# tomisetsu/mochi-db

Hardware: AMD Instinct MI355X
Metric: verified grant signatures/sec (1/2/4/8 GPU) + % of INT32 VALU roofline (higher is better)
Workload: dtype u32

## Files before the change

mochi-db_amd/csrc/kara_dev.h:

```cpp
#pragma once
#include "fold.h"
#include "mont.h"

namespace mochi {

constexpr int kKH = kL / 2;
static_assert(2 * kKH == kL, "even limb count");

template <int AO, int BO, int K, int NA, int NB>
__device__ __forceinline__ uint32_t product_col(const uint32_t (&a)[NA], const uint32_t (&b)[NB], uint64_t& carry) {
  if constexpr (K == 2 * kKH - 1) {
    return (uint32_t)carry & kLimbMask;
  } else if constexpr (K == 2 * kKH) {
    return (uint32_t)(carry >> kLimbBits);
  } else {
    constexpr int lo = K - kKH + 1 > 0 ? K - kKH + 1 : 0;
    constexpr int hi = K < kKH - 1 ? K : kKH - 1;
    uint64_t acc = carry;
    static_for<lo, hi + 1>([&](auto ic) {
      constexpr int i = decltype(ic)::value;
      acc = mad64(a[AO + i], b[BO + K - i], acc);
      asm volatile("" ::"v"(acc));
    });
    carry = acc >> kLimbBits;
    return (uint32_t)acc & kLimbMask;
  }
}

template <int AO, int K, int NA>
__device__ __forceinline__ uint32_t square_col(uint32_t (&a)[NA], uint64_t& carry) {
  if constexpr (K == 2 * kKH - 1) {
    return (uint32_t)carry & kLimbMask;
  } else if constexpr (K == 2 * kKH) {
    return (uint32_t)(carry >> kLimbBits);
  } else {
    constexpr int lo = K - kKH + 1 > 0 ? K - kKH + 1 : 0;
    constexpr int xhi = K > 0 ? (K - 1) / 2 : -1;
    uint64_t acc = carry;
    static_for<lo, xhi + 1>([&](auto ic) {
      constexpr int i = decltype(ic)::value;
      acc = mad64(a[AO + i], a[AO + K - i], acc);
      asm volatile("" ::"v"(acc));
    });
    if constexpr ((K & 1) == 0) {
      acc = mad64(a[AO + (K >> 1)], a[AO + (K >> 1)], acc);
      if constexpr ((K >> 1) < kKH - 1) a[AO + (K >> 1)] += a[AO + (K >> 1)];
    }
    carry = acc >> kLimbBits;
    return (uint32_t)acc & kLimbMask;
  }
}

template <typename COL>
__device__ __forceinline__ void kara_middle(uint32_t (&t)[2 * kL], COL&& col) {
  uint64_t carry = 0;
  static_for<0, 2 * kKH + 1>([&](auto kc) {
    constexpr int k = decltype(kc)::value;
    t[kKH + k] = col(kc, carry);
    __builtin_amdgcn_sched_barrier(0);
  });
}

template <typename LOW, typename HIGH>
__device__ __forceinline__ void kara_combine(uint32_t (&t)[2 * kL], LOW&& low, HIGH&& high) {
  uint64_t cl = 0, ch = 0;
  static_for<0, 3 * kKH>([&](auto cc) {
    constexpr int c = decltype(cc)::value;
    if constexpr (c < kKH) {
      const uint32_t l = low(cc, cl);
      t[c] = l;
      t[kKH + c] -= l;
    } else if constexpr (c < kL) {
      const uint32_t l = low(cc, cl);
      const uint32_t h = high(std::integral_constant<int, c - kKH>{}, ch);
      const uint32_t q = l - h;
      t[c] += q;
      if constexpr (c >= kFoldF) t[c] ^= kFoldBias;
      t[kKH + c] -= q;
    } else {
      constexpr int m = c - kKH;
      const uint32_t h = high(std::integral_constant<int, m>{}, ch);
      t[c] -= h;
      t[c] ^= kFoldBias;
      if constexpr (m == kKH) {
        t[kKH + c] += h;
        t[kKH + c] ^= kFoldBias;
      } else {
        t[kKH + c] = h ^ kFoldBias;
      }
    }
    __builtin_amdgcn_sched_barrier(0);
  });
}

__device__ __forceinline__ void kara_square(uint32_t (&x)[kL], uint32_t (&t)[2 * kL]) {
  {
    uint32_t sx[kKH];
#pragma unroll
    for (int i = 0; i < kKH; i++) sx[i] = x[i] + x[kKH + i];
    kara_middle(t, [&](auto kc, uint64_t& carry) { return square_col<0, decltype(kc)::value>(sx, carry); });
  }
  kara_combine(
      t, [&](auto kc, uint64_t& carry) { return square_col<0, decltype(kc)::value>(x, carry); },
      [&](auto kc, uint64_t& carry) { return square_col<kKH, decltype(kc)::value>(x, carry); });
}

#ifndef MOCHI_KARA2
#define MOCHI_KARA2 0
#endif

template <int AO, int K, int N, int NA>
__device__ __forceinline__ uint32_t square_col_n(uint32_t (&a)[NA], uint64_t& carry) {
  if constexpr (K == 2 * N - 1) {
    return (uint32_t)carry & kLimbMask;
  } else if constexpr (K == 2 * N) {
    return (uint32_t)(carry >> kLimbBits);
  } else {
    constexpr int lo = K - N + 1 > 0 ? K - N + 1 : 0;
    constexpr int xhi = K > 0 ? (K - 1) / 2 : -1;
    uint64_t acc = carry;
    static_for<lo, xhi + 1>([&](auto ic) {
      constexpr int i = decltype(ic)::value;
      acc = mad64(a[AO + i], a[AO + K - i], acc);
      asm volatile("" ::"v"(acc));
    });
    if constexpr ((K & 1) == 0) {
      acc = mad64(a[AO + (K >> 1)], a[AO + (K >> 1)], acc);
      if constexpr ((K >> 1) < N - 1) a[AO + (K >> 1)] += a[AO + (K >> 1)];
    }
    carry = acc >> kLimbBits;
    return (uint32_t)acc & kLimbMask;
  }
}

template <int AO, int NA>
struct Square2 {
  static constexpr int N0 = 19, N1 = kKH - N0;
  uint32_t (&a)[NA];
  uint32_t s[N0];
  int32_t r[N0];
  uint64_t c0 = 0, c1 = 0, c2 = 0;
  int32_t cn = 0;
  __device__ __forceinline__ explicit Square2(uint32_t (&x)[NA]) : a(x) {
#pragma unroll
    for (int i = 0; i < N0; i++) s[i] = a[AO + i] + (i < N1 ? a[AO + N0 + i] : 0u);
  }
  template <int C>
  __device__ __forceinline__ uint32_t col() {
    int32_t p0 = 0, p1 = 0, p2 = 0;
    if constexpr (C <= 2 * N0) p0 = (int32_t)square_col_n<AO, C, N0>(a, c0);
    if constexpr (C - N0 >= 0 && C - N0 <= 2 * N1) p1 = (int32_t)square_col_n<AO + N0, C - N0, N1>(a, c1);
    if constexpr (C - N0 >= 0 && C - N0 <= 2 * N0) p2 = (int32_t)square_col_n<0, C - N0, N0>(s, c2);
    const int32_t rc = p0 - p1;
    int32_t v = rc + p2 + cn;
    if constexpr (C >= N0) v -= r[C % N0];
    r[C % N0] = rc;
    cn = v >> kLimbBits;
    return (uint32_t)v & kLimbMask;
  }
};

__device__ __forceinline__ void kara_square2_lockstep(uint32_t (&x)[kL], uint32_t (&t)[2 * kL]) {
  {
    uint32_t sx[kKH];
#pragma unroll
    for (int i = 0; i < kKH; i++) sx[i] = x[i] + x[kKH + i];
    kara_middle(t, [&](auto kc, uint64_t& carry) { return square_col<0, decltype(kc)::value>(sx, carry); });
  }
  Square2<0, kL> lo(x);
#if MOCHI_KARA2 == 5
  Square2<kKH, kL> hi(x);
  kara_combine(
      t, [&](auto kc, uint64_t&) { return lo.template col<decltype(kc)::value>(); },
      [&](auto kc, uint64_t&) { return hi.template col<decltype(kc)::value>(); });
#else
  kara_combine(
      t, [&](auto kc, uint64_t&) { return lo.template col<decltype(kc)::value>(); },
      [&](auto kc, uint64_t& carry) { return square_col<kKH, decltype(kc)::value>(x, carry); });
#endif
}

__device__ __forceinline__ void kara_square2(uint32_t (&x)[kL], uint32_t (&t)[2 * kL]) {
  {
    uint32_t sx[kKH];
#pragma unroll
    for (int i = 0; i < kKH; i++) sx[i] = x[i] + x[kKH + i];
    kara_middle(t, [&](auto kc, uint64_t& carry) { return square_col<0, decltype(kc)::value>(sx, carry); });
  }
  {
#if MOCHI_KARA2 == 3
    uint64_t cl = 0;
#else
    Square2<0, kL> lo(x);
#endif
    static_for<0, kL>([&](auto cc) {
      constexpr int c = decltype(cc)::value;
#if MOCHI_KARA2 == 3
      const uint32_t l = square_col<0, c>(x, cl);
#else
      const uint32_t l = lo.template col<c>();
#endif
      if constexpr (c < kKH) t[c] = l;
      else t[c] += l;
      t[kKH + c] -= l;
      __builtin_amdgcn_sched_barrier(0);
    });
  }
  {
#if MOCHI_KARA2 >= 2
    uint64_t ch = 0;
#else
    Square2<kKH, kL> hi(x);
#endif
    static_for<0, kL>([&](auto mc) {
      constexpr int m = decltype(mc)::value;
#if MOCHI_KARA2 >= 2
      const uint32_t h = square_col<kKH, m>(x, ch);
#else
      const uint32_t h = hi.template col<m>();
#endif
      t[kKH + m] -= h;
      if constexpr (m <= kKH) t[kL + m] += h;
      else t[kL + m] = h;
      __builtin_amdgcn_sched_barrier(0);
    });
  }
#pragma unroll
  for (int k = kFoldF; k < 2 * kL; k++) t[k] ^= kFoldBias;
}

__device__ __forceinline__ void kara_product(const uint32_t (&x)[kL], const uint32_t (&y)[kL], uint32_t (&t)[2 * kL]) {
  {
    uint32_t sx[kKH], sy[kKH];
#pragma unroll
    for (int i = 0; i < kKH; i++) {
      sx[i] = x[i] + x[kKH + i];
      sy[i] = y[i] + y[kKH + i];
    }
    kara_middle(t, [&](auto kc, uint64_t& carry) { return product_col<0, 0, decltype(kc)::value>(sx, sy, carry); });
  }
  kara_combine(
      t, [&](auto kc, uint64_t& carry) { return product_col<0, 0, decltype(kc)::value>(x, y, carry); },
      [&](auto kc, uint64_t& carry) { return product_col<kKH, kKH, decltype(kc)::value>(x, y, carry); });
}

}
```

mochi-db_amd/csrc/rsa_final.hip:

```cpp
#include "fold_dev.h"
#include "rsa_common.h"

#include <cstdlib>

#ifndef MOCHI_FINAL_DYN
#define MOCHI_FINAL_DYN 0
#endif

#ifndef MOCHI_FINAL_STAMPS
#define MOCHI_FINAL_STAMPS 0
#endif

namespace mochi {
#if MOCHI_FINAL_STAMPS
__device__ unsigned long long g_final_stamps[4096][6];
#endif
namespace {

struct FStamps {
  uint64_t load = 0, prod = 0, fold = 0, check = 0, n = 0;
};

__device__ __forceinline__ uint64_t fstamp() {
#if MOCHI_FINAL_STAMPS
  __builtin_amdgcn_sched_barrier(0);
  const uint64_t t = __builtin_amdgcn_s_memtime();
  __builtin_amdgcn_sched_barrier(0);
  return t;
#else
  return 0;
#endif
}

#ifndef MOCHI_FINAL_WAIT
#define MOCHI_FINAL_WAIT 1
#endif

struct FinalOps {
  uint4 sr[16];
  uint32_t z[kL];
  uint32_t hw[8];
  uint32_t g, fl, d;
};

__device__ __forceinline__ void final_load(uint32_t slot, uint32_t g_lead, const uint32_t* __restrict__ perm,
                                           uint32_t n_slots, const uint8_t* __restrict__ sig,
                                           const uint32_t* __restrict__ zin, const uint32_t* __restrict__ lead,
                                           const uint8_t* __restrict__ flags, FinalOps& o) {
  o.g = slot < n_slots ? perm[slot] : 0xFFFFFFFFu;
  const uint32_t gg = o.g != 0xFFFFFFFFu ? o.g : g_lead;
  o.d = lead ? lead[gg] : gg;
  o.fl = flags[gg];
  const uint4* s128 = (const uint4*)(sig + (size_t)gg * MOCHI_RSA_BYTES);
#pragma unroll
  for (int q = 0; q < 16; q++) o.sr[q] = s128[q];
  const gchar* zp = (const gchar*)zin;
  const uint32_t zoff = slot * 4u;
  const size_t zstride = (size_t)n_slots * 4u;
#pragma unroll
  for (int j = 0; j < kL; j++) {
    o.z[j] = *(const guint*)(zp + zoff);
    zp += zstride;
    asm volatile("" : "+s"(zp));
  }
}

__device__ __forceinline__ void final_load_digest(const uint32_t* __restrict__ digest, uint32_t n_dist, FinalOps& o) {
#pragma unroll
  for (int i = 0; i < 8; i++) o.hw[i] = digest[(size_t)(7 - i) * n_dist + o.d];
}

__device__ __forceinline__ void final_slot(FinalOps& o, uint32_t key, uint32_t g_lead,
                                           const KeyEntry* __restrict__ keys, const FoldKey* __restrict__ fold,
                                           const uint32_t* __restrict__ digest, const uint32_t* __restrict__ lead,
                                           uint32_t n_dist, uint8_t* __restrict__ flags, const v4i* w,
                                           FStamps& st) {
  const uint32_t g = o.g;
  const bool active = g != 0xFFFFFFFFu;
  if (__ballot(active) == 0) return;
  const uint64_t t1 = fstamp();
  const KeyEntry* ke = keys + key;
  const cptr n = as_const(ke->n);
  uint32_t sv[kL];
  {
    uint32_t wd[64];
#pragma unroll
    for (int q = 0; q < 16; q++) {
      wd[63 - 4 * q] = bswap32(o.sr[q].x);
      wd[62 - 4 * q] = bswap32(o.sr[q].y);
      wd[61 - 4 * q] = bswap32(o.sr[q].z);
      wd[60 - 4 * q] = bswap32(o.sr[q].w);
    }
    words_to_limbs(wd, sv);
  }
  int32_t br = 0;
#pragma unroll
  for (int j = 0; j < kL; j++) br = ((int32_t)sv[j] - (int32_t)n[j] - br) < 0 ? 1 : 0;
  asm volatile("" : "+v"(br));
  const bool s_lt_n = br != 0;
  uint32_t (&x)[kL] = o.z;
  uint32_t t[2 * kL];
  kara_product(x, sv, t);
  const uint64_t t2 = fstamp();
  uint32_t hl[kHL];
  {
    const uint32_t (&hw)[8] = o.hw;
#pragma unroll
    for (int j = 0; j < kHL; j++) {
      const int bit = j * kLimbBits, wi = bit >> 5, sh = bit & 31;
      const uint64_t v = ((uint64_t)(wi + 1 < 8 ? hw[wi + 1] : 0u) << 32) | hw[wi];
      hl[j] = (uint32_t)(v >> sh) & kLimbMask;
    }
  }
  fold_reduce<true, true>(t, x, w + (threadIdx.x & 63), as_const(fold[key].cnc), hl);
  const uint64_t t3 = fstamp();
  cptr nn = n;
  asm volatile("" : "+s"(nn));
  const uint32_t n0inv = *as_const(&ke->n0inv);
  const uint32_t m = (x[0] * n0inv) & kLimbMask;
  uint64_t c = mad64(m, nn[0], x[0]) >> kLimbBits;
  uint32_t diff = 0;
#pragma unroll
  for (int k = 1; k < kL; k++) {
    const uint64_t acc = mad64(m, nn[k], x[k] + c);
    diff |= ((uint32_t)acc & kLimbMask) ^ nn[k - 1];
    c = acc >> kLimbBits;
  }
  diff |= c != (uint64_t)nn[kL - 1] ? 1u : 0u;
  if (active) {
    const bool ok = s_lt_n && diff == 0;
    flags[g] = (uint8_t)(o.fl | (ok ? MOCHI_GRANT_SIG_OK : 0));
  }
#if MOCHI_FINAL_STAMPS
  const uint64_t t4 = fstamp();
  st.prod += t2 - t1;
  st.fold += t3 - t2;
  st.check += t4 - t3;
  st.n++;
#else
  (void)t1, (void)t2, (void)t3, (void)st;
#endif
}

__global__ __launch_bounds__(256, 1) void k_rsa_final(const uint32_t* __restrict__ perm, uint32_t n_slots,
                                                       const uint8_t* __restrict__ sig,
                                                       const uint16_t* __restrict__ signer,
                                                       const KeyEntry* __restrict__ keys,
                                                       const FoldKey* __restrict__ fold,
                                                       const uint32_t* __restrict__ zin,
                                                       const uint32_t* __restrict__ digest,
                                                       const uint32_t* __restrict__ lead, uint32_t n_dist,
                                                       uint8_t* __restrict__ flags, uint32_t* __restrict__ ctr) {
  __shared__ v4i w[kFoldImgBytes / 16];
  FStamps st;
  const uint64_t t_begin = fstamp();
  for_groups(perm, n_slots, signer, fold, w, [&](uint32_t base, uint32_t key, uint32_t g_lead) {
#pragma unroll 1
    for (uint32_t h = 0; h < kBucketAlign; h += 256) {
      FinalOps o;
      const uint64_t t0 = fstamp();
      final_load(base + h + threadIdx.x, g_lead, perm, n_slots, sig, zin, lead, flags, o);
#if MOCHI_FINAL_STAMPS == 2 || (MOCHI_FINAL_WAIT && !MOCHI_FINAL_STAMPS)
      asm volatile("s_waitcnt vmcnt(0)" ::: "memory");
#endif
      final_load_digest(digest, n_dist, o);
#if MOCHI_FINAL_STAMPS
      st.load += fstamp() - t0;
#endif
      (void)t0;
      final_slot(o, key, g_lead, keys, fold, digest, lead, n_dist, flags, w, st);
    }
  }, MOCHI_FINAL_DYN ? ctr : nullptr);
#if MOCHI_FINAL_STAMPS
  const uint64_t t_end = fstamp();
  const uint32_t wv = (blockIdx.x * blockDim.x + threadIdx.x) >> 6;
  if ((threadIdx.x & 63) == 0 && wv < 4096) {
    g_final_stamps[wv][0] = st.load;
    g_final_stamps[wv][1] = st.prod;
    g_final_stamps[wv][2] = st.fold;
    g_final_stamps[wv][3] = st.check;
    g_final_stamps[wv][4] = st.n;
    g_final_stamps[wv][5] = t_end - t_begin;
  }
#else
  (void)t_begin;
#endif
}

__global__ __launch_bounds__(256, 1) void k_rsa_final_lat(const uint32_t* __restrict__ perm, uint32_t n_slots,
                                                           const uint8_t* __restrict__ sig,
                                                           const uint16_t* __restrict__ signer,
                                                           const KeyEntry* __restrict__ keys,
                                                           const FoldKey* __restrict__ fold,
                                                           const uint32_t* __restrict__ zin,
                                                           const uint32_t* __restrict__ digest,
                                                           const uint32_t* __restrict__ lead, uint32_t n_dist,
                                                           uint8_t* __restrict__ flags) {
  __shared__ v4i w[kFoldImgBytes / 16];
  __shared__ uint32_t xr[kLatRows][kLatChunk];
  const uint32_t wv = __builtin_amdgcn_readfirstlane(threadIdx.x >> 6), lane = threadIdx.x & 63;
  const uint32_t base = blockIdx.x * kLatChunk;
  if (base >= n_slots) return;
  const uint32_t g_lead = __builtin_amdgcn_readfirstlane(perm[base]);
  if (g_lead == 0xFFFFFFFFu) return;
  const uint32_t key = __builtin_amdgcn_readfirstlane((uint32_t)signer[g_lead]);
  {
    const v4i* src = (const v4i*)fold[key].img;
    for (uint32_t i = threadIdx.x; i < kFoldImgBytes / 16; i += blockDim.x) w[i] = src[i];
  }
  const bool two = __builtin_amdgcn_readfirstlane(base + 32 < n_slots && perm[base + 32] != 0xFFFFFFFFu);
  const uint32_t slot = base + lane;
  const uint32_t g = slot < n_slots ? perm[slot] : 0xFFFFFFFFu;
  const bool active = g != 0xFFFFFFFFu;
  const uint32_t gg = active ? g : g_lead;
  const uint32_t fl = flags[gg];
  uint32_t z[kL], sv[kL];
#pragma unroll
  for (int j = 0; j < kL; j++) z[j] = zin[(size_t)j * n_slots + (slot < n_slots ? slot : base)];
  {
    uint32_t wd[64];
    load_sig_words(sig, gg, wd);
    words_to_limbs(wd, sv);
  }
  __syncthreads();
  uint32_t lv[kL];
  if (wv == 0) {
    uint64_t carry = 0;
    static_for<0, kL>([&](auto kc) {
      constexpr int k = decltype(kc)::value;
      lv[k] = product_col<0, 0, k>(z, sv, carry);
    });
  } else if (wv == 1) {
    uint32_t hv[kL];
    uint64_t carry = 0;
    static_for<0, kL>([&](auto kc) {
      constexpr int k = decltype(kc)::value;
      hv[k] = product_col<kKH, kKH, k>(z, sv, carry);
    });
#pragma unroll
    for (int k = 0; k < kL; k++) xr[k][lane] = hv[k];
  } else if (wv == 2) {
    uint32_t sz[kKH], ss[kKH];
#pragma unroll
    for (int i = 0; i < kKH; i++) {
      sz[i] = z[i] + z[kKH + i];
      ss[i] = sv[i] + sv[kKH + i];
    }
    uint32_t mv[kL + 1];
    uint64_t carry = 0;
    static_for<0, kL + 1>([&](auto kc) {
      constexpr int k = decltype(kc)::value;
      mv[k] = product_col<0, 0, k>(sz, ss, carry);
    });
#pragma unroll
    for (int k = 0; k <= kL; k++) xr[kL + k][lane] = mv[k];
  }
  __syncthreads();
  if (wv == 0) {
    uint32_t t[2 * kL], hv[kL];
#pragma unroll
    for (int k = 0; k <= kL; k++) t[kKH + k] = xr[kL + k][lane];
#pragma unroll
    for (int k = 0; k < kL; k++) hv[k] = xr[k][lane];
    kara_combine(
        t, [&](auto kc, uint64_t&) { return lv[decltype(kc)::value]; },
        [&](auto kc, uint64_t&) { return hv[decltype(kc)::value]; });
#pragma unroll
    for (int k = 0; k < 2 * kL; k++) xr[k][lane] = t[k];
  }
  uint32_t hl[kHL];
  {
    const uint32_t d = lead ? lead[gg] : gg;
    uint32_t hw[8];
#pragma unroll
    for (int i = 0; i < 8; i++) hw[i] = digest[(size_t)(7 - i) * n_dist + d];
#pragma unroll
    for (int j = 0; j < kHL; j++) {
      const int bit = j * kLimbBits, wi = bit >> 5, sh = bit & 31;
      const uint64_t v = ((uint64_t)(wi + 1 < 8 ? hw[wi + 1] : 0u) << 32) | hw[wi];
      hl[j] = (uint32_t)(v >> sh) & kLimbMask;
    }
  }
  __syncthreads();
  const v4i* wl = w + lane;
  cptr cn = as_const(fold[key].cnc);
  asm volatile("" : "+s"(cn));
  if (two) {
    if (wv == 0) lat_fold<0, true, true>(wl, cn, xr, lane, hl);
    else if (wv == 1) lat_fold<1, true, true>(wl, cn, xr, lane, hl);
    else if (wv == 2) lat_fold<2, true, true>(wl, cn, xr, lane, hl);
    else lat_fold<3, true, true>(wl, cn, xr, lane, hl);
  } else {
    if (wv == 0) lat_fold<0, false, true>(wl, cn, xr, lane, hl);
    else if (wv == 1) lat_fold<1, false, true>(wl, cn, xr, lane, hl);
    else if (wv == 2) lat_fold<2, false, true>(wl, cn, xr, lane, hl);
    else lat_fold<3, false, true>(wl, cn, xr, lane, hl);
  }
  __syncthreads();
  if (wv != 0) return;
  uint32_t x[kL];
  {
    int pq[2 * kL];
#pragma unroll
    for (int i = 0; i < 2 * kL; i++) pq[i] = (int)xr[i][lane];
    int64_t carry = 0;
#pragma unroll
    for (int q = 0; q < kL; q++) {
      const int64_t v = mad_i64(pq[2 * q + 1], 65536, mad_i64(pq[2 * q], 1, carry));
      x[q] = (uint32_t)v & kLimbMask;
      carry = v >> kLimbBits;
    }
  }
  const KeyEntry* ke = keys + key;
  const cptr n = as_const(ke->n);
  int32_t br = 0;
#pragma unroll
  for (int j = 0; j < kL; j++) br = ((int32_t)sv[j] - (int32_t)n[j] - br) < 0 ? 1 : 0;
  const uint32_t n0inv = *as_const(&ke->n0inv);
  const uint32_t m = (x[0] * n0inv) & kLimbMask;
  uint64_t c = mad64(m, n[0], x[0]) >> kLimbBits;
  uint32_t diff = 0;
#pragma unroll
  for (int k = 1; k < kL; k++) {
    const uint64_t acc = mad64(m, n[k], x[k] + c);
    diff |= ((uint32_t)acc & kLimbMask) ^ n[k - 1];
    c = acc >> kLimbBits;
  }
  diff |= c != (uint64_t)n[kL - 1] ? 1u : 0u;
  if (active) {
    const bool ok = br != 0 && diff == 0;
    flags[g] = (uint8_t)(fl | (ok ? MOCHI_GRANT_SIG_OK : 0));
  }
}

static bool final_lat_off() {
  static const bool off = [] {
    const char* e = getenv("MOCHI_NO_FINAL_LAT");
    return e && e[0] == '1';
  }();
  return off;
}

}

void launch_rsa_final(const LaunchArgs& a, const uint32_t* lead, uint32_t n_dist, hipStream_t st, bool latency) {
  if (a.dbg_y) {
    launch_rsa_raw(a, st);
    return;
  }
  if (latency && !final_lat_off()) {
    const uint32_t chunks = (a.n_slots + kLatChunk - 1) / kLatChunk;
    if (chunks)
      hipLaunchKernelGGL(k_rsa_final_lat, dim3(chunks), dim3(256), 0, st, a.perm, a.n_slots, a.sig, a.signer, a.keys,
                         a.fold, a.xbuf, a.digest, lead, n_dist, a.flags);
    return;
  }
  const uint32_t blocks = fold_grid(a.n_slots);
  if (!blocks) return;
  hipLaunchKernelGGL(k_rsa_final, dim3(blocks), dim3(256), 0, st, a.perm, a.n_slots, a.sig, a.signer, a.keys, a.fold,
                     a.xbuf, a.digest, lead, n_dist, a.flags, a.total + kTotFinalGroup);
}

}

#if MOCHI_FINAL_STAMPS
extern "C" int mochi_debug_final_stamps(unsigned long long* out, unsigned n_waves) {
  if (n_waves > 4096) n_waves = 4096;
  return hipMemcpyFromSymbol(out, HIP_SYMBOL(mochi::g_final_stamps), 48 * (size_t)n_waves, 0, hipMemcpyDeviceToHost) ==
                 hipSuccess
             ? 0
             : -1;
}
#endif
```

Measured before the change: 366.8 million.

## Split final RSA kernel into two phase-staggered wave groups with LDS-parked limbs

Replaces the final verification kernel with a 512-thread version. Two halves of the block run staggered with barriers, so one half's Karatsuba low/high product overlaps the other's fold-reduce and check. To cut register pressure, the low product limbs are parked in LDS rows through inline ds_write/ds_read with immediate offsets and reloaded before folding. The kernel also uses static contiguous group assignment per block instead of the dynamic counter and prefetches the next group's key, at the cost of extra barriers, more LDS use, and sensitivity to kBucketAlign matching the block size.

```diff
diff --git a/mochi-db_amd/csrc/kara_dev.h b/mochi-db_amd/csrc/kara_dev.h
--- a/mochi-db_amd/csrc/kara_dev.h
+++ b/mochi-db_amd/csrc/kara_dev.h
@@ -244,4 +244,101 @@
       [&](auto kc, uint64_t& carry) { return product_col<kKH, kKH, decltype(kc)::value>(x, y, carry); });
 }
 
-}
+constexpr int kParkLimbs = 28;
+constexpr int kParkStride = (int)kBucketAlign * 4;
+static_assert(kParkLimbs % 7 == 0 && kParkLimbs <= kKH, "parked limbs are read back seven at a time");
+static_assert((kParkLimbs - 1) * kParkStride < 65536, "row offsets fit the DS instruction's immediate");
+
+template <int ROW>
+__device__ __forceinline__ void park_put(uint32_t park, uint32_t v) {
+  asm volatile("ds_write_b32 %0, %1 offset:%2" ::"v"(park), "v"(v), "n"(ROW * kParkStride) : "memory");
+}
+
+template <int R0>
+__device__ __forceinline__ void park_get7(uint32_t park, uint32_t (&v)[7]) {
+  asm volatile(
+      "ds_read_b32 %0, %7 offset:%8\n\t"
+      "ds_read_b32 %1, %7 offset:%9\n\t"
+      "ds_read_b32 %2, %7 offset:%10\n\t"
+      "ds_read_b32 %3, %7 offset:%11\n\t"
+      "ds_read_b32 %4, %7 offset:%12\n\t"
+      "ds_read_b32 %5, %7 offset:%13\n\t"
+      "ds_read_b32 %6, %7 offset:%14\n\t"
+      "s_waitcnt lgkmcnt(0)"
+      : "=&v"(v[0]), "=&v"(v[1]), "=&v"(v[2]), "=&v"(v[3]), "=&v"(v[4]), "=&v"(v[5]), "=&v"(v[6])
+      : "v"(park), "n"(R0 * kParkStride), "n"((R0 + 1) * kParkStride), "n"((R0 + 2) * kParkStride),
+        "n"((R0 + 3) * kParkStride), "n"((R0 + 4) * kParkStride), "n"((R0 + 5) * kParkStride),
+        "n"((R0 + 6) * kParkStride)
+      : "memory");
+}
+
+__device__ __forceinline__ void park_reload(uint32_t park, uint32_t (&t)[2 * kL]) {
+  static_for<0, kParkLimbs / 7>([&](auto bc) {
+    constexpr int b = decltype(bc)::value;
+    uint32_t v[7];
+    park_get7<7 * b>(park, v);
+#pragma unroll
+    for (int j = 0; j < 7; j++) t[7 * b + j] = v[j];
+  });
+}
+
+__device__ __forceinline__ void kara_consume_lh(uint32_t (&x)[kL], uint32_t (&y)[kL], uint32_t (&t)[2 * kL],
+                                                uint32_t park) {
+  {
+    uint64_t cl = 0, ch = 0;
+    static_for<0, kL>([&](auto cc) {
+      constexpr int c = decltype(cc)::value;
+      uint32_t l = product_col<0, 0, c>(x, y, cl);
+      uint32_t h = product_col<kKH, kKH, c>(x, y, ch);
+      asm volatile("" : "+v"(l), "+v"(h));
+      if constexpr (c < kParkLimbs) park_put<c>(park, l);
+      else t[c] = l;
+      t[kL + c] = h;
+      if constexpr (c >= kKH - 1 && c - (kKH - 1) < kKH) {
+        constexpr int i = c - (kKH - 1);
+        x[i] += x[kKH + i];
+        y[i] += y[kKH + i];
+      }
+      __builtin_amdgcn_sched_barrier(0);
+    });
+  }
+  static_for<kKH, kL>([&](auto kc) {
+    constexpr int k = decltype(kc)::value;
+    constexpr int j = k - kKH;
+    const uint32_t q = t[k] - t[k + kKH];
+    t[k + kKH] = 0u - q - t[k + kL];
+    if constexpr (k + kL > kKH + kL) t[k + kL] ^= kFoldBias;
+    if constexpr (j >= kParkLimbs) t[k] = q - t[j];
+    else t[k] = q;
+    asm volatile("" : "+v"(t[k]), "+v"(t[k + kKH]), "+v"(t[k + kL]));
+  });
+  static_for<0, kParkLimbs / 7>([&](auto bc) {
+    constexpr int b = decltype(bc)::value;
+    uint32_t v[7];
+    park_get7<7 * b>(park, v);
+#pragma unroll
+    for (int j = 0; j < 7; j++) t[kKH + 7 * b + j] -= v[j];
+  });
+  __builtin_amdgcn_sched_barrier(0);
+}
+
+__device__ __forceinline__ void kara_consume_m(uint32_t (&x)[kL], uint32_t (&y)[kL], uint32_t (&t)[2 * kL]) {
+  {
+    uint64_t cm = 0;
+    static_for<0, 2 * kKH + 1>([&](auto mc) {
+      constexpr int m = decltype(mc)::value;
+      t[kKH + m] += product_col<0, 0, m>(x, y, cm);
+      if constexpr (kKH + m >= kFoldF) t[kKH + m] ^= kFoldBias;
+      asm volatile("" : "+v"(t[kKH + m]));
+      __builtin_amdgcn_sched_barrier(0);
+    });
+  }
+}
+
+__device__ __forceinline__ void kara_product_consume(uint32_t (&x)[kL], uint32_t (&y)[kL], uint32_t (&t)[2 * kL],
+                                                     uint32_t park) {
+  kara_consume_lh(x, y, t, park);
+  kara_consume_m(x, y, t);
+}
+
+}
diff --git a/mochi-db_amd/csrc/rsa_final.hip b/mochi-db_amd/csrc/rsa_final.hip
--- a/mochi-db_amd/csrc/rsa_final.hip
+++ b/mochi-db_amd/csrc/rsa_final.hip
@@ -9,6 +9,10 @@
 
 #ifndef MOCHI_FINAL_STAMPS
 #define MOCHI_FINAL_STAMPS 0
+#endif
+
+#ifndef MOCHI_FINAL_TWO
+#define MOCHI_FINAL_TWO 1
 #endif
 
 namespace mochi {
@@ -43,6 +47,7 @@
   uint32_t g, fl, d;
 };
 
+template <bool FLAGS = true>
 __device__ __forceinline__ void final_load(uint32_t slot, uint32_t g_lead, const uint32_t* __restrict__ perm,
                                            uint32_t n_slots, const uint8_t* __restrict__ sig,
                                            const uint32_t* __restrict__ zin, const uint32_t* __restrict__ lead,
@@ -50,7 +55,7 @@
   o.g = slot < n_slots ? perm[slot] : 0xFFFFFFFFu;
   const uint32_t gg = o.g != 0xFFFFFFFFu ? o.g : g_lead;
   o.d = lead ? lead[gg] : gg;
-  o.fl = flags[gg];
+  if constexpr (FLAGS) o.fl = flags[gg];
   const uint4* s128 = (const uint4*)(sig + (size_t)gg * MOCHI_RSA_BYTES);
 #pragma unroll
   for (int q = 0; q < 16; q++) o.sr[q] = s128[q];
@@ -70,6 +75,7 @@
   for (int i = 0; i < 8; i++) o.hw[i] = digest[(size_t)(7 - i) * n_dist + o.d];
 }
 
+#if !MOCHI_FINAL_TWO
 __device__ __forceinline__ void final_slot(FinalOps& o, uint32_t key, uint32_t g_lead,
                                            const KeyEntry* __restrict__ keys, const FoldKey* __restrict__ fold,
                                            const uint32_t* __restrict__ digest, const uint32_t* __restrict__ lead,
@@ -142,6 +148,183 @@
 #endif
 }
 
+#endif
+
+#if MOCHI_FINAL_TWO
+__device__ __forceinline__ uint32_t lane_id() {
+  uint32_t tid = threadIdx.x;
+  asm volatile("" : "+v"(tid));
+  return tid;
+}
+
+__device__ __forceinline__ void final_fold_check(uint32_t (&t)[2 * kL], const FinalOps& o, uint32_t key,
+                                                 const KeyEntry* __restrict__ keys, const FoldKey* __restrict__ fold,
+                                                 uint8_t* __restrict__ flags, const v4i* w, uint32_t park,
+                                                 FStamps& st) {
+  const uint64_t t2 = fstamp();
+  uint32_t hl[kHL];
+#pragma unroll
+  for (int j = 0; j < kHL; j++) {
+    const int bit = j * kLimbBits, wi = bit >> 5, sh = bit & 31;
+    const uint64_t v = ((uint64_t)(wi + 1 < 8 ? o.hw[wi + 1] : 0u) << 32) | o.hw[wi];
+    hl[j] = (uint32_t)(v >> sh) & kLimbMask;
+  }
+  park_reload(park, t);
+  uint32_t x[kL];
+  fold_reduce<true, true>(t, x, w + (lane_id() & 63), as_const(fold[key].cnc), hl);
+  const uint64_t t3 = fstamp();
+  const KeyEntry* ke = keys + key;
+  cptr nn = as_const(ke->n);
+  asm volatile("" : "+s"(nn));
+  const uint32_t n0inv = *as_const(&ke->n0inv);
+  const uint32_t m = (x[0] * n0inv) & kLimbMask;
+  uint64_t c = mad64(m, nn[0], x[0]) >> kLimbBits;
+  uint32_t diff = 0;
+#pragma unroll
+  for (int k = 1; k < kL; k++) {
+    const uint64_t acc = mad64(m, nn[k], x[k] + c);
+    diff |= ((uint32_t)acc & kLimbMask) ^ nn[k - 1];
+    c = acc >> kLimbBits;
+  }
+  diff |= c != (uint64_t)nn[kL - 1] ? 1u : 0u;
+  if (o.g != 0xFFFFFFFFu) {
+    flags[o.g] = (uint8_t)(o.fl | (diff == 0 ? MOCHI_GRANT_SIG_OK : 0));
+  }
+#if MOCHI_FINAL_STAMPS
+  st.fold += t3 - t2;
+  st.check += fstamp() - t3;
+  st.n++;
+#else
+  (void)t2, (void)t3, (void)st;
+#endif
+}
+
+__device__ __forceinline__ void phase_barrier() {
+  __builtin_amdgcn_sched_barrier(0);
+  __builtin_amdgcn_s_barrier();
+  __builtin_amdgcn_sched_barrier(0);
+}
+
+__global__ __launch_bounds__(512, 1) void k_rsa_final(const uint32_t* __restrict__ perm, uint32_t n_slots,
+                                                       const uint8_t* __restrict__ sig,
+                                                       const uint16_t* __restrict__ signer,
+                                                       const KeyEntry* __restrict__ keys,
+                                                       const FoldKey* __restrict__ fold,
+                                                       const uint32_t* __restrict__ zin,
+                                                       const uint32_t* __restrict__ digest,
+                                                       const uint32_t* __restrict__ lead, uint32_t n_dist,
+                                                       uint8_t* __restrict__ flags, uint32_t* __restrict__ ctr) {
+  __shared__ v4i w[kFoldImgBytes / 16];
+  __shared__ uint32_t park_rows[kParkLimbs * kBucketAlign];
+  FStamps st;
+  const uint64_t t_begin = fstamp();
+  auto park_of = [&](uint32_t tid) {
+    return (uint32_t)(uintptr_t)(__attribute__((address_space(3))) uint32_t*)(park_rows + tid);
+  };
+  const bool lag = __builtin_amdgcn_readfirstlane(threadIdx.x >> 6) >= 4;
+  const uint32_t n_groups = (n_slots + kBucketAlign - 1) / kBucketAlign;
+  uint32_t grp = (uint32_t)((uint64_t)blockIdx.x * n_groups / gridDim.x);
+  const uint32_t g_end = (uint32_t)((uint64_t)(blockIdx.x + 1) * n_groups / gridDim.x);
+  uint32_t g_lead = 0xFFFFFFFFu;
+  while (grp < g_end && (g_lead = __builtin_amdgcn_readfirstlane(perm[grp * kBucketAlign])) == 0xFFFFFFFFu) grp++;
+  if (grp >= g_end) return;
+  uint32_t key = __builtin_amdgcn_readfirstlane((uint32_t)signer[g_lead]);
+  auto stage = [&](uint32_t k) {
+    typedef __attribute__((address_space(1))) v4i gv4i;
+    const gchar* src = (const gchar*)fold[k].img;
+#pragma unroll 1
+    for (uint32_t i = lane_id(); i < kFoldImgBytes / 16; i += kBucketAlign) w[i] = *(const gv4i*)(src + i * 16u);
+    __syncthreads();
+  };
+  stage(key);
+  if (lag) phase_barrier();
+  bool key_changed = false;
+  for (;;) {
+    if (!lag && key_changed) {
+      phase_barrier();
+      stage(key);
+    }
+    FinalOps o;
+    final_load<false>(grp * kBucketAlign + threadIdx.x, g_lead, perm, n_slots, sig, zin, lead, flags, o);
+    uint32_t nxt = grp + 1, n_lead = 0xFFFFFFFFu;
+    while (nxt < g_end && (n_lead = __builtin_amdgcn_readfirstlane(perm[nxt * kBucketAlign])) == 0xFFFFFFFFu) nxt++;
+    const bool more = nxt < g_end;
+    const uint32_t n_key = more ? __builtin_amdgcn_readfirstlane((uint32_t)signer[n_lead]) : key;
+    const uint64_t t0 = fstamp();
+    asm volatile("s_waitcnt vmcnt(0)" ::: "memory");
+    const uint64_t t1 = fstamp();
+    if (__ballot(o.g != 0xFFFFFFFFu) != 0) {
+      uint32_t sv[kL];
+      {
+        uint32_t wd[64];
+#pragma unroll
+        for (int q = 0; q < 16; q++) {
+          wd[63 - 4 * q] = bswap32(o.sr[q].x);
+          wd[62 - 4 * q] = bswap32(o.sr[q].y);
+          wd[61 - 4 * q] = bswap32(o.sr[q].z);
+          wd[60 - 4 * q] = bswap32(o.sr[q].w);
+        }
+        words_to_limbs(wd, sv);
+      }
+      const cptr n = as_const(keys[key].n);
+      int32_t br = 0;
+#pragma unroll
+      for (int j = 0; j < kL; j++) br = ((int32_t)sv[j] - (int32_t)n[j] - br) < 0 ? 1 : 0;
+      if (br == 0) o.g = 0xFFFFFFFFu;
+      asm volatile("" : "+v"(o.g));
+      uint32_t t[2 * kL];
+      kara_consume_lh(o.z, sv, t, park_of(lane_id()));
+      final_load_digest(digest, n_dist, o);
+      o.fl = flags[o.g != 0xFFFFFFFFu ? o.g : g_lead];
+#if MOCHI_FINAL_STAMPS
+      st.load += t1 - t0;
+      st.prod += fstamp() - t1;
+#endif
+      __builtin_amdgcn_sched_barrier(0);
+      phase_barrier();
+      const uint64_t t1m = fstamp();
+      kara_consume_m(o.z, sv, t);
+#if MOCHI_FINAL_STAMPS
+      st.prod += fstamp() - t1m;
+#else
+      (void)t1m;
+#endif
+      __builtin_amdgcn_s_setprio(1);
+      final_fold_check(t, o, key, keys, fold, flags, w, park_of(lane_id()), st);
+      __builtin_amdgcn_s_setprio(0);
+    } else {
+      phase_barrier();
+    }
+    (void)t0, (void)t1;
+    phase_barrier();
+    if (!more) break;
+    if (lag && n_key != key) {
+      stage(n_key);
+      phase_barrier();
+    }
+    key_changed = n_key != key;
+    grp = nxt;
+    key = n_key;
+    g_lead = n_lead;
+  }
+  if (!lag) phase_barrier();
+#if MOCHI_FINAL_STAMPS
+  const uint64_t t_end = fstamp();
+  const uint32_t wv = (blockIdx.x * blockDim.x + threadIdx.x) >> 6;
+  if ((threadIdx.x & 63) == 0 && wv < 4096) {
+    g_final_stamps[wv][0] = st.load;
+    g_final_stamps[wv][1] = st.prod;
+    g_final_stamps[wv][2] = st.fold;
+    g_final_stamps[wv][3] = st.check;
+    g_final_stamps[wv][4] = st.n;
+    g_final_stamps[wv][5] = t_end - t_begin;
+  }
+#else
+  (void)t_begin;
+#endif
+  (void)ctr;
+}
+#else
 __global__ __launch_bounds__(256, 1) void k_rsa_final(const uint32_t* __restrict__ perm, uint32_t n_slots,
                                                        const uint8_t* __restrict__ sig,
                                                        const uint16_t* __restrict__ signer,
@@ -187,6 +370,8 @@
 #endif
 }
 
+#endif
+
 __global__ __launch_bounds__(256, 1) void k_rsa_final_lat(const uint32_t* __restrict__ perm, uint32_t n_slots,
                                                            const uint8_t* __restrict__ sig,
                                                            const uint16_t* __restrict__ signer,
@@ -357,7 +542,7 @@
   }
   const uint32_t blocks = fold_grid(a.n_slots);
   if (!blocks) return;
-  hipLaunchKernelGGL(k_rsa_final, dim3(blocks), dim3(256), 0, st, a.perm, a.n_slots, a.sig, a.signer, a.keys, a.fold,
+  hipLaunchKernelGGL(k_rsa_final, dim3(blocks), dim3(MOCHI_FINAL_TWO ? kBucketAlign : 256), 0, st, a.perm, a.n_slots, a.sig, a.signer, a.keys, a.fold,
                      a.xbuf, a.digest, lead, n_dist, a.flags, a.total + kTotFinalGroup);
 }
 
```

Result: no change. 369.3 million (median of 6 runs) (+0.7%).
